# askerlee/AdaFace-dev

Measured on AMD Instinct MI355X. Metric: denoise-steps/sec SD-1.5 U-Net 512px bs=4/GPU, higher is better.
Workload: dtype f16; 1 GPU; adaface_txt2img_ddim: SD-1.5 U-Net eps-prediction + CFG + DDIM update, 512x512 (latent 64x64), bs=4/GPU, U-Net batch 8 (cond+uncond), 77 tokens, DDIM-50 timesteps, random-init weights; parallelism=replicas x1, hipgraph=True, finite=True

## Files before the change

adaface-dev_amd/_lib.py:

```python
import ctypes as C
import os
import subprocess

_HERE = os.path.dirname(os.path.abspath(__file__))
CSRC = os.path.join(_HERE, "csrc")
LIB_PATH = os.environ.get("AF_LIB") or os.path.join(CSRC, "libadaface_hip.so")

AF_OK, AF_E_BADARG, AF_E_UNSUPPORTED, AF_E_HIP = 0, -1, -2, -3
AF_ACT_NONE, AF_ACT_SILU, AF_ACT_GEGLU, AF_ACT_QUICKGELU = 0, 1, 2, 3
AF_OUT_NORMAL, AF_OUT_SPLIT_T, AF_OUT_F32 = 0, 1, 2
AF_SPLITK_COUNTER_BYTES = 4096 * 4
AF_FAM_GEMM, AF_FAM_ATTN, AF_FAM_GNORM, AF_FAM_LNORM, AF_FAM_ELEM, AF_FAM_XATTN = 0, 1, 2, 3, 4, 5

EXPORTS = (
    "af_last_error", "af_version", "af_device_count", "af_prof_enable", "af_prof_reset", "af_prof_read",
    "af_gemm", "af_groupnorm_ws_floats", "af_groupnorm", "af_layernorm", "af_attention", "af_attention_scores",
    "af_timestep_embedding", "af_nchw_f32_to_nhwc_f16", "af_nhwc_f16_to_nchw_f32", "af_cfg_ddim_step", "af_q_sample",
    "af_silu_f16", "af_attention_lse", "af_groupnorm_stats", "af_attention_bwd_scratch_bytes", "af_attention_bwd",
    "af_groupnorm_bwd", "af_layernorm_bwd", "af_geglu_fwd", "af_geglu_bwd", "af_sumpool2x2", "af_add_f16",
    "af_transpose_tokens", "af_cadamw_step", "af_attention_ex", "af_colsum", "af_quickgelu_fwd", "af_quickgelu_bwd",
    "af_scale_f32", "af_affine_prelu", "af_maxpool2x2", "af_global_avgpool", "af_se_residual_prelu", "af_axpy_f16", "af_dora_combine", "af_mul_f16", "af_im2col3x3", "af_colsum_tall", "af_softmax_rows", "af_attention_strided", "af_clamp_f32", "af_mask_pairs", "af_prefetch", "af_prefetch_ex",
    "af_xattn_scores", "af_xattn_softmax_pv", "af_xattn_softmax_pv_bwd", "af_xattn_rowmix", "af_xattn_colmix_ws_bytes", "af_xattn_colmix",
    "af_layernorm_param_grads", "af_transpose_tokens_pair", "af_ff_fused", "af_ff_chain", "af_xattn_fused",
    "af_softmax_rows_bwd", "af_affine_prelu_bwd", "af_maxpool2x2_bwd", "af_se_gate_grad", "af_se_residual_prelu_bwd",
    "af_groupnorm_apply", "af_gemm_gn_stats_ok", "af_gemm_halo_variant", "af_gn_proj_fused",
    "af_splitk_reduce", "af_groupnorm_splitk_ok", "af_groupnorm_splitk", "af_xattn_chain",
    "af_image_u8_to_nhwc_f16", "af_vae_latents_q_sample", "af_cfg_dpmpp_step", "af_cfg_lcm_step",
    "af_cfg_ddim_inpaint_step", "af_cfg_dpmpp_inpaint_step", "af_cfg_lcm_inpaint_step", "af_vae_latents_z_q_sample",
    "af_vae_attention", "af_latent_resize_q_sample", "af_affine_prelu_ch", "af_face_align_crop",
    "af_stem_im2col7x7", "af_relu_maxpool3x3s2", "af_subsample2x", "af_upsample2x_add", "af_retina_decode", "af_retina_nms",
)


class GemmDesc(C.Structure):
    _fields_ = [
        ("a1", C.c_void_p), ("a2", C.c_void_p), ("wt", C.c_void_p), ("bias", C.c_void_p),
        ("rowbias", C.c_void_p), ("residual", C.c_void_p), ("out", C.c_void_p), ("out2", C.c_void_p),
        ("M", C.c_int32), ("N", C.c_int32), ("K", C.c_int32), ("kpad", C.c_int32), ("taps", C.c_int32),
        ("c1", C.c_int32), ("c2", C.c_int32), ("lda1", C.c_int32), ("lda2", C.c_int32),
        ("B", C.c_int32), ("H", C.c_int32), ("W", C.c_int32), ("Ho", C.c_int32), ("Wo", C.c_int32),
        ("stride", C.c_int32), ("upsample", C.c_int32), ("rows_per_batch", C.c_int32), ("ld_rowbias", C.c_int32),
        ("act", C.c_int32), ("out_mode", C.c_int32), ("ld_out", C.c_int32), ("split_col", C.c_int32),
        ("ld_out2", C.c_int32), ("tile", C.c_int32), ("splits", C.c_int32),
        ("workspace", C.c_void_p), ("workspace_bytes", C.c_int64), ("zeros", C.c_void_p),
        ("tap_shift", C.c_int32), ("splitk_fused", C.c_int32),
        ("ln_colsum", C.c_void_p), ("ln_eps", C.c_float),
        ("a3", C.c_void_p), ("a4", C.c_void_p), ("c3", C.c_int32), ("c4", C.c_int32), ("lda3", C.c_int32), ("lda4", C.c_int32),
        ("gn_partials", C.c_void_p), ("gn_cpg", C.c_int32),
        ("defer_reduce", C.POINTER(C.c_int32)),
    ]


def _csrc_sha() -> str:
    import glob
    import hashlib
    h = hashlib.sha256()
    files = sorted(glob.glob(os.path.join(CSRC, "*.hip")) + glob.glob(os.path.join(CSRC, "*.h")))
    files += [os.path.join(CSRC, "Makefile"), os.path.join(os.path.dirname(_HERE), "include", "adaface_hip.h")]
    for f in files:
        h.update(os.path.basename(f).encode())
        with open(f, "rb") as fh:
            h.update(fh.read())
    return h.hexdigest()
# ... 25 lines not shown

_lib = None


def lib() -> C.CDLL:
    global _lib
    if _lib is not None:
        return _lib
    import torch
    if not os.path.exists(LIB_PATH):
        raise RuntimeError(
            f"{LIB_PATH} not found: the HIP extension is required (no CPU fallback). "
            "Run `python -c 'import __graft_entry__ as g; g.build()'` or `make -C adaface-dev_amd/csrc`."
        )
    L = C.CDLL(LIB_PATH)
    vp, i32, i64, f32 = C.c_void_p, C.c_int, C.c_int64, C.c_float
    L.af_last_error.restype = C.c_char_p
    L.af_last_error.argtypes = []
    L.af_version.argtypes = []
    L.af_device_count.argtypes = []
    L.af_prof_enable.argtypes = [i32]
    L.af_prof_reset.argtypes = []
    L.af_prof_read.argtypes = [i32, C.POINTER(C.c_int), C.POINTER(C.c_double)]
    L.af_gemm.argtypes = [C.POINTER(GemmDesc), vp]
    L.af_groupnorm_ws_floats.argtypes = [i32]
    L.af_groupnorm.argtypes = [vp, vp, i32, i32, vp, vp, vp, i32, i32, i32, f32, i32, vp, vp]
    L.af_groupnorm_apply.argtypes = [vp, i32, vp, vp, vp, vp, i32, i32, i32, f32, i32, vp, i32, vp]
    L.af_gemm_gn_stats_ok.argtypes = [i32, i32, i32, i32, i32, i32, i32, i32]
    L.af_gemm_halo_variant.argtypes = [C.POINTER(GemmDesc)]
    L.af_splitk_reduce.argtypes = [vp, i32, vp, vp, i32, i32, vp, vp, i32, i32, vp]
    L.af_groupnorm_splitk_ok.argtypes = [i32, i32, i32, i32]
    L.af_groupnorm_splitk.argtypes = [vp, i32, vp, vp, i32, vp, vp, i32, vp, vp, vp, vp, i32, i32, i32, f32, i32, vp]
    L.af_gn_proj_fused.argtypes = [vp, vp, i32, vp, vp, f32, vp, vp, i32, vp, i32, i32, i32, i32, vp, vp]
    L.af_layernorm.argtypes = [vp, vp, vp, vp, i32, i32, f32, vp]
    L.af_attention.argtypes = [vp, vp, vp, vp, vp, i32, i32, i32, i32, i32, i32, i32, i32, i32, i32, f32, vp]
    L.af_attention_scores.argtypes = [vp, vp, vp, vp, i32, i32, i32, i32, i32, f32, vp]
    L.af_timestep_embedding.argtypes = [vp, vp, i32, i32, f32, vp]
    L.af_nchw_f32_to_nhwc_f16.argtypes = [vp, vp, i32, i32, i32, i32, vp]
    L.af_nhwc_f16_to_nchw_f32.argtypes = [vp, vp, i32, i32, i32, i32, vp]
    L.af_cfg_ddim_step.argtypes = [vp, vp, vp, vp, i64, i32, f32, f32, f32, vp]
    L.af_cfg_dpmpp_step.argtypes = [vp, vp, vp, vp, vp, vp, i64, i32, f32, f32, f32, f32, f32, f32, vp]
    L.af_cfg_lcm_step.argtypes = [vp, vp, vp, vp, vp, i64, i32, f32, f32, f32, f32, f32, f32, f32, vp]
    L.af_q_sample.argtypes = [vp, vp, vp, vp, vp, i32, i64, vp]
    L.af_image_u8_to_nhwc_f16.argtypes = [vp, vp, i32, i32, i32, vp]
    L.af_vae_latents_q_sample.argtypes = [vp, vp, vp, vp, vp, f32, f32, f32, vp, i32, i32, i32, i32, vp]
    L.af_vae_latents_z_q_sample.argtypes = [vp, vp, vp, vp, vp, f32, f32, f32, vp, vp, i32, i32, i32, i32, vp]
    L.af_latent_resize_q_sample.argtypes = [vp, vp, vp, i32, i32, i32, i32, i32, i32, f32, f32, vp]
    blend = [vp, vp, vp, i32, i32, i64, f32, f32]
    L.af_cfg_ddim_inpaint_step.argtypes = L.af_cfg_ddim_step.argtypes[:-1] + blend + [vp]
    L.af_cfg_dpmpp_inpaint_step.argtypes = L.af_cfg_dpmpp_step.argtypes[:-1] + blend + [vp]
    L.af_cfg_lcm_inpaint_step.argtypes = L.af_cfg_lcm_step.argtypes[:-1] + blend + [vp]
    L.af_silu_f16.argtypes = [vp, vp, i64, vp]
    L.af_attention_lse.argtypes = [vp, vp, vp, vp, vp, i32, vp, i32, i32, i32, i32, i32, i32, i32, i32, i32, i32, f32, vp]
    L.af_attention_ex.argtypes = [vp, vp, vp, vp, vp, i32, vp, i32, i32, i32, i32, i32, i32, i32, i32, i32, i32, i32, f32, vp]
    L.af_attention_strided.argtypes = [vp, vp, vp, vp, vp, i32, vp, i32, i32, i32, i32, i32, i32, i32, i32, i32, i32, i32, i64, f32, vp]
    L.af_groupnorm_stats.argtypes = [vp, vp, i32, i32, vp, vp, vp, vp, i32, i32, i32, f32, i32, vp, vp]
    L.af_attention_bwd_scratch_bytes.argtypes = [i32, i32, i32, i32, i32]
    L.af_attention_bwd.argtypes = [vp, vp, vp, vp, vp, vp, i32, vp, i32, vp, vp, vp, vp, i64] + [i32] * 14 + [f32, vp]
    L.af_axpy_f16.argtypes = [vp, vp, f32, vp, i64, vp]
    L.af_dora_combine.argtypes = [vp, vp, vp, vp, vp, vp, i64, i32, vp]
    L.af_mul_f16.argtypes = [vp, vp, vp, i64, vp]
    L.af_im2col3x3.argtypes = [vp, vp, i32, i32, i32, i32, i32, vp]
    L.af_softmax_rows.argtypes = [vp, vp, i64, i32, vp]
    L.af_mask_pairs.argtypes = [vp, vp, i32, vp]
    L.af_vae_attention.argtypes = [vp, vp, vp, vp, i32, i32, i32, i32, i32, i32, i32, vp]
    L.af_prefetch.argtypes = [vp, i64, vp]
# ... 58 lines not shown
```

adaface-dev_amd/ldm/modules/diffusionmodules/openaimodel.py:

```python
import os
from abc import abstractmethod

import torch
import torch.nn as nn

from .... import ops
from ....ops import AF_ACT_SILU, F16
from ..attention import SpatialTransformer
from .util import (_PackCache, checkpoint, conv_nd, from_nhwc_f16, linear, normalization, timestep_embedding,
                   to_nhwc_f16, zero_module)


class TimestepBlock(nn.Module):
    @abstractmethod
    def forward(self, x, emb):
        """Apply the module to `x` given `emb` timestep embeddings."""


FUSE_SKIP = os.environ.get("AF_FUSE_SKIP", "1") != "0"


class SkipCat(tuple):
    """(h, skip): the decoder's channel concat, kept as two tensors so consumers read both
    sources directly instead of materialising torch.cat (openaimodel.py:918)."""


class EmbPack:

    def __init__(self, silu_emb, all_out=None):
        self.silu_emb = silu_emb
        self.all_out = all_out


class TimestepEmbedSequential(nn.Sequential, TimestepBlock):
    def hip(self, x, emb, context=None, mask=None):
        n = len(self)
        for i, layer in enumerate(self):
            if isinstance(layer, ResBlock):
                x = layer.hip(x, emb, defer_out=i + 1 < n and isinstance(self[i + 1], SpatialTransformer))
            elif isinstance(layer, TimestepBlock):
                x = layer.hip(x, emb)
            elif isinstance(layer, SpatialTransformer):
                x = layer.hip(x, context, mask)
            else:
                x = layer.hip(x)
        return x

    def hip_train(self, x, emb, context=None, mask=None):
        saved = []
        for layer in self:
            if isinstance(layer, TimestepBlock):
                x, s = layer.hip_train(x, emb)
# ... 349 lines not shown
        ca_idx = self.ALL_CA_LAYER_INDICES if ca_layer_indices is None else ca_layer_indices
        tr_idx = self.ALL_CA_LAYER_INDICES if trans_layer_indices is None else trans_layer_indices
        return apply(ca_flag_dict, ca_idx, "ca"), apply(trans_flag_dict, tr_idx, "trans")

    def _packed_emb_all(self):
        params = []
        for rb in self._resblocks:
            params += [rb.emb_layers[1].weight, rb.emb_layers[1].bias]

        def build():
            dev = params[0].device
            K = self._resblocks[0].emb_channels
            w = torch.zeros((self._emb_total, K), dtype=torch.float32, device=dev)
            b = torch.zeros((self._emb_total,), dtype=torch.float32, device=dev)
            for rb in self._resblocks:
                off, width = rb._emb_slice
                w[off:off + width] = rb.emb_layers[1].weight.detach().float()
                b[off:off + width] = rb.emb_layers[1].bias.detach().float()
            return ops.pack_matrix(w, b, dev)

        return self._emb_cache.get(params, build)

    def prepare(self):
        for m in self.modules():
            if hasattr(m, "packed"):
                m.packed()
            if hasattr(m, "_packed_qkv") and m.to_k.in_features == m.to_q.in_features:
                m._packed_qkv()
            if hasattr(m, "_packed_kv") and m.to_k.in_features != m.to_q.in_features:
                m._packed_kv()
        self._packed_emb_all()
        return self

    def hip(self, x_nhwc, timesteps, context, img_mask=None, capture_layers=()):
        emb = self._embed(timesteps)
        kv_layers = self._project_context_all(context)
        try:
            return self._hip_blocks(x_nhwc, emb, context, img_mask, capture_layers)
        finally:
            for m in kv_layers:
                m._kv_pre = None

    def _cross_attn_layers(self):
        out = []
        for blocks in (self.input_blocks, [self.middle_block], self.output_blocks):
            for module in blocks:
                for layer in module:
                    if isinstance(layer, SpatialTransformer):
                        out += [tb.attn2 for tb in layer.transformer_blocks]
        return out

    def _project_context_all(self, context):
        layers = self._cross_attn_layers()
        if not layers or context is None:
            return []
        ws = [m.to_k.weight for m in layers] + [m.to_v.weight for m in layers]
        if not hasattr(self, "_kv_all_cache"):
            self._kv_all_cache = _PackCache()
        pack = self._kv_all_cache.get(ws, lambda: ops.pack_matrix(torch.cat([w.detach() for w in ws], 0), None, ws[0].device))
        B, L, cc = context.shape
        sc = pack.N // 2
        k_all, vt_all = ops.gemm(context.reshape(B * L, cc), pack, rows_per_batch=L, split_col=sc)
        off = 0
        for m in layers:
            c = m.inner_dim
            m._kv_pre = (k_all[:, off:off + c], vt_all[:, off:off + c, :], sc)
            off += c
        return layers

    def _hip_blocks(self, x_nhwc, emb, context, img_mask, capture_layers):
        acts = {}
        hs = []
        h = x_nhwc
        layer_idx = 0

        def collect(module, h):
            attn2 = module[1].transformer_blocks[0].attn2
            a = attn2.cached_activations
            a["outfeat"] = from_nhwc_f16(h, torch.float32)
            acts[layer_idx] = a
            attn2.cached_activations = None

        for module in self.input_blocks:
            h = module.hip(h, emb, context, img_mask)
            hs.append(h)
            if layer_idx in capture_layers:
                collect(module, h)
            layer_idx += 1
        h = self.middle_block.hip(h, emb, context, img_mask)
        if layer_idx in capture_layers:
            collect(self.middle_block, h)
        layer_idx += 1
        for module in self.output_blocks:
            h = module.hip(SkipCat((h, hs.pop())), emb, context, img_mask)
            if layer_idx in capture_layers:
                collect(module, h)
            layer_idx += 1
        h = self.out[0].hip(h, silu=True)
        return self.out[2].hip(h), acts

    def hip_tail(self, trunk, timesteps, context, capture_layers, n_tail=3):
        h, skips = trunk
        emb = self._embed(timesteps)
        kv_layers = self._project_context_all(context)
        acts = {}
        try:
            n_out = len(self.output_blocks)
            layer_idx = len(self.input_blocks) + 1 + n_out - n_tail
            for k, module in enumerate(list(self.output_blocks)[n_out - n_tail:]):
                h = module.hip(SkipCat((h, skips[k])), emb, context, None)
                if layer_idx in capture_layers:
                    attn2 = module[1].transformer_blocks[0].attn2
                    a = attn2.cached_activations
                    a["outfeat"] = from_nhwc_f16(h, torch.float32)
                    acts[layer_idx] = a
                    attn2.cached_activations = None
                layer_idx += 1
            h = self.out[0].hip(h, silu=True)
            return self.out[2].hip(h), acts
        finally:
            for m in kv_layers:
                m._kv_pre = None

    def _embed(self, timesteps):
        t_emb = timestep_embedding(timesteps, self.model_channels)
        e0 = ops.gemm(t_emb, self.time_embed[0].packed(), act=AF_ACT_SILU)
        semb = ops.gemm(e0, self.time_embed[2].packed(), act=AF_ACT_SILU)
        return EmbPack(semb, ops.gemm(semb, self._packed_emb_all()))

    def hip_train(self, x_nhwc, timesteps, context, img_mask=None):
        emb = self._embed(timesteps)
        saved_in, saved_out, hs = [], [], []
        h = x_nhwc
        for module in self.input_blocks:
            h, s = module.hip_train(h, emb, context, img_mask)
            saved_in.append(s)
            hs.append(h)
        h, saved_mid = self.middle_block.hip_train(h, emb, context, img_mask)
        for module in self.output_blocks:
            h, s = module.hip_train(SkipCat((h, hs.pop())), emb, context, img_mask)
            saved_out.append(s)
        g, st = self.out[0].hip_train(h, silu=True)
        return self.out[2].hip(g), (saved_in, saved_mid, saved_out, h, st, context.shape)

    def hip_train_trunk(self, x_nhwc, emb, context, img_mask, n_tail):
        saved_in, saved_out, hs = [], [], []
        h = x_nhwc
        for module in self.input_blocks:
            h, s = module.hip_train(h, emb, context, img_mask)
            saved_in.append(s)
            hs.append(h)
        h, saved_mid = self.middle_block.hip_train(h, emb, context, img_mask)
# ... 58 lines not shown
            scaled = res_gradscale != 1.0 and (n_out - 1 - i) >= self.num_res_blocks + 1
            d = ops.axpy(d, dskips[i], res_gradscale) if scaled else ops.add(d, dskips[i])
            if i == 0 and not need_dx:
                return None, dctx.reshape(ctx_shape)
            d, dctx = self.input_blocks[i].hip_bwd(saved_in[i], d, dctx)
        return d, dctx.reshape(ctx_shape)

    def forward(self, x, timesteps=None, context=None, y=None, context_in=None, extra_info=None, **kwargs):
        assert y is None, "must specify y if and only if the model is class-conditional"
        capture = extra_info.get("capture_ca_activations", False) if extra_info is not None else False
        img_mask = extra_info.get("img_mask", None) if extra_info is not None else None
        captured = [22, 23, 24] if capture else []
        old_flags = None
        if capture:
            old_flags, _ = self.set_cross_attn_flags(ca_flag_dict={"save_cross_attn_vars": True}, ca_layer_indices=captured)
        ei = extra_info or {}
        rewrites = bool(ei.get("normalize_cross_attn", False) or ei.get("mix_attn_mats_in_batch", False))
        trainable = torch.is_grad_enabled() and (x.requires_grad or context.requires_grad or ei.get("_ffn_lora_adapters")
                                                 or ei.get("_attn_lora_adapters"))
        if rewrites or ei.get("_attn_lora_adapters") or (capture and trainable):
            from .capture_graph import unet_forward_captured
            if extra_info is None:
                raise ValueError("extra_info must be a dict on the capture / score-rewrite path")
            if capture:
                self.set_cross_attn_flags(ca_flag_dict=old_flags, ca_layer_indices=captured)
            eps = unet_forward_captured(self, x, timesteps, context, extra_info)
            if not capture:
                extra_info.pop("ca_layers_activations", None)
            return eps
        if trainable:
            gs = float((extra_info or {}).get("res_hidden_states_gradscale", 1) or 1)
            lora = (extra_info or {}).get("_ffn_lora_adapters")
            return _UNetFunction.apply(self, x, timesteps, context, img_mask, gs, lora, *[t[3] for t in lora_param_order(lora)])
        try:
            ctx = context.to(F16).contiguous()
            shared = None
            if img_mask is None and ei.get("_trunk_cache") is not None:
                from .capture_graph import cached_trunk
                shared = cached_trunk(ei, x.shape[0])
            if shared is not None:
                eps, acts = self.hip_tail(shared, timesteps, ctx, captured)
            else:
                xh = to_nhwc_f16(x, ops.round_up(self.in_channels, 8))
                eps, acts = self.hip(xh, timesteps, ctx, img_mask, captured)
        finally:
            if capture:
                self.set_cross_attn_flags(ca_flag_dict=old_flags, ca_layer_indices=captured)
        if extra_info is not None:
            extra_info["ca_layers_activations"] = {
                key: {li: acts[li][key] for li in acts} for key in ("outfeat", "attn", "attnscore", "q", "q2", "k", "v", "attn_out")
            }
        return from_nhwc_f16(eps, x.dtype, self.out_channels)


class _UNetFunction(torch.autograd.Function):

    @staticmethod
    def forward(ctx, unet, x, timesteps, context, img_mask, res_gradscale=1.0, lora=None, *lora_params):
        ctx.res_gradscale = res_gradscale
        ctx.lora = lora
        ctx.need_dx, ctx.x_dtype, ctx.c_dtype = x.requires_grad, x.dtype, context.dtype

        def body(xs, ts, cs, ms):
            xh = to_nhwc_f16(xs, ops.round_up(unet.in_channels, 8))
            try:
                for bi, ads in (lora or {}).items():
                    unet.output_blocks[bi][0]._lora = ads
                eps, saved = unet.hip_train(xh, ts, cs.to(F16).contiguous(), ms)
            finally:
                for bi in (lora or {}):
                    unet.output_blocks[bi][0]._lora = None
            return from_nhwc_f16(eps, xs.dtype, unet.out_channels), saved

        graphs = getattr(unet, "train_graphs", None)
        if graphs is not None and x.is_cuda:
            ctx.key = (tuple(x.shape), tuple(context.shape), str(x.dtype), str(context.dtype), img_mask is not None, float(res_gradscale),
                       tuple(id(a) for _, _, _, a in lora_param_order(lora)), ctx.need_dx)
            from_graph = not graphs[0].busy(ctx.key) and graphs[0].entries.get(ctx.key, {}).get("state") in ("warm", "graph")
            out, ctx.saved = graphs[0].run(ctx.key, body, [x.detach(), timesteps, context.detach(), img_mask],
                                           refresh=lambda: _refresh_adapter_packs(lora))
            if not from_graph:
                ctx.key = None
            elif any(ctx.needs_input_grad):
                graphs[0].claim(ctx.key, ctx)
# ... 54 lines not shown
```

adaface-dev_amd/ops.py:

```python
import ctypes as C
from dataclasses import dataclass
from typing import Optional

import torch

from . import _lib
from ._lib import AF_ACT_GEGLU, AF_ACT_NONE, AF_ACT_QUICKGELU, AF_ACT_SILU, AF_OUT_F32, AF_OUT_NORMAL, AF_OUT_SPLIT_T, GemmDesc

F16 = torch.float16
NEG_MAX = -torch.finfo(torch.float32).max



def param_key(p):
    if p is None:
        return None
    gen = p.__dict__.get("_af_gen")
    return (p.data_ptr(), p._version, p.device, gen[0] if gen is not None else -1)


def _stream() -> int:
    return torch._C._cuda_getCurrentRawStream(torch._C._cuda_getDevice())


# ... 576 lines not shown
        rc = _lib.lib().af_groupnorm(_p(x), _p(x2), c1, c2, _p(gamma), _p(beta), _p(y), B, hw, groups, float(eps), int(silu), _p(ws), _stream())
        _lib.check(rc, "af_groupnorm")
    else:
        rc = _lib.lib().af_groupnorm_stats(_p(x), _p(x2), c1, c2, _p(gamma), _p(beta), _p(y), _p(stats), B, hw, groups, float(eps), int(silu), _p(ws), _stream())
        _lib.check(rc, "af_groupnorm_stats")
    return y, stats


def groupnorm(x: torch.Tensor, gamma: torch.Tensor, beta: torch.Tensor, eps: float, silu: bool, *,
              x2: Optional[torch.Tensor] = None, groups: int = 32) -> torch.Tensor:
    return _groupnorm(x, gamma, beta, eps, silu, x2, groups, False)[0]


def groupnorm_train(x, gamma, beta, eps, silu, *, x2=None, groups=32):
    return _groupnorm(x, gamma, beta, eps, silu, x2, groups, True)


def gn_proj_fused(x: torch.Tensor, gamma: torch.Tensor, beta: torch.Tensor, eps: float, pw: PackedWeight, groups: int = 32) -> Optional[torch.Tensor]:
    gn = partials_of(x)
    B, c = x.shape[0], x.shape[-1]
    hw = x.numel() // (B * c)
    if (gn is None or c != 320 or groups != 32 or pw.N != 320 or pw.K != 320 or pw.ln_cs is not None or hw % 128 != 0 or gn.B != B or gn.hw != hw or gn.C != c
            or gn.cpg * groups != c or not x.is_contiguous()):
        return None
    _chk_f16(x, "gn_proj_fused.x")
    out = torch.empty((B * hw, pw.N), dtype=F16, device=x.device)
    _pf_note(pw.wt)
    rc = _lib.lib().af_gn_proj_fused(_p(x), _p(gn.ws), gn.nblk, _p(gamma), _p(beta), float(eps), _p(pw.wt), _p(pw.bias), pw.kpad, _p(out), B, hw, c, groups,
                                     _zero_page(x.device).data_ptr(), _stream())
    _lib.check(rc, "af_gn_proj_fused")
    return out


def layernorm(x: torch.Tensor, gamma: torch.Tensor, beta: torch.Tensor, eps: float = 1e-5) -> torch.Tensor:
    _chk_f16(x, "layernorm.x")
    Cn = x.shape[-1]
    y = torch.empty_like(x)
    _lib.check(_lib.lib().af_layernorm(_p(x), _p(gamma), _p(beta), _p(y), x.numel() // Cn, Cn, float(eps), _stream()),
               "af_layernorm")
    return y


def attention(q: torch.Tensor, k: torch.Tensor, vt: torch.Tensor, *, B: int, Nq: int, L: int, heads: int, d: int,
              ldq: int, ldk: int, keybias: Optional[torch.Tensor] = None, scale: Optional[float] = None,
              want_lse: bool = False, causal_m: int = 0):
    Cn = heads * d
    o = torch.empty((B * Nq, Cn), dtype=F16, device=q.device)
    scale = d ** -0.5 if scale is None else scale
    ldb = 0 if keybias is None else keybias.stride(0)
    lse = torch.empty((B, heads, round_up(Nq, 32)), dtype=torch.float32, device=q.device) if want_lse else None
    rc = _lib.lib().af_attention_strided(_p(q), _p(k), _p(vt), _p(o), _p(lse), 0 if lse is None else lse.stride(1), _p(keybias),
                                         int(causal_m), B, Nq, L, heads, d, ldq, ldk, Cn, vt.stride(1), ldb, vt.stride(0), float(scale),
                                         _stream())
    _lib.check(rc, "af_attention")
    return (o, lse) if want_lse else o


_attn_scratch = {}


def attention_bwd(q, k, v, o, dout, lse, *, B: int, Nq: int, L: int, heads: int, d: int, ldq: int, ldk: int, ldv: int,
                  dq: torch.Tensor, dk: torch.Tensor, dv: torch.Tensor, lddq: int, lddk: int, lddv: int,
                  keybias: Optional[torch.Tensor] = None, scale: Optional[float] = None, causal_m: int = 0):
    Cn = heads * d
    scale = d ** -0.5 if scale is None else scale
    need = _lib.lib().af_attention_bwd_scratch_bytes(B, Nq, L, heads, d)
# ... 631 lines not shown
```

include/adaface_hip.h:

```cpp
#ifndef ADAFACE_HIP_H
#define ADAFACE_HIP_H

#include <stdint.h>

#ifdef __cplusplus
extern "C" {
#endif

#define AF_OK 0
#define AF_E_BADARG (-1)
#define AF_E_UNSUPPORTED (-2)
#define AF_E_HIP (-3)

const char* af_last_error(void);
int af_version(void);
int af_device_count(void);

#define AF_FAM_GEMM 0
#define AF_FAM_ATTN 1
#define AF_FAM_GNORM 2
#define AF_FAM_LNORM 3
#define AF_FAM_ELEM 4
#define AF_FAM_XATTN 5
#define AF_FAM_COUNT 6
// ... 47 lines not shown
  const void* a4;
  int32_t c3, c4, lda3, lda4;
  void* gn_partials;
  int32_t gn_cpg;
  int32_t* defer_reduce;
} af_gemm_desc;
#define AF_SPLITK_MAX_TILES 4096
#define AF_SPLITK_COUNTER_BYTES (AF_SPLITK_MAX_TILES * 4)

int af_gemm(const af_gemm_desc* d, void* stream);

int af_splitk_reduce(const void* slabs, int splits, const void* bias, const void* rowbias, int ld_rowbias, int rows_per_batch, const void* residual,
                     void* out, int M, int N, void* stream);

int af_ff_fused(const void* x, const void* w1, const void* b1, const void* ln_colsum, float ln_eps, int kpad1, const void* w2, const void* b2,
                int kpad2, const void* residual, void* out, int M, int C, int inner, const void* zeros, void* stream);
int af_ff_chain(const void* x, const void* w1, const void* b1, const void* ln_colsum, float ln_eps, int kpad1, const void* w2, const void* b2, int kpad2,
                const void* residual, const void* wp, const void* bp, int kpad_p, const void* x_in, void* out, void* gn_partials, int gn_cpg,
                int rows_per_batch, int M, int C, int inner, const void* zeros, void* stream);

int af_xattn_fused(const void* x, const void* wq, const void* bq, const void* ln_colsum, float ln_eps, int kpad_q, const void* k, int ldk,
                   const void* vt, int64_t vt_batch_stride, int ldv, const void* wo, const void* bo, int kpad_o, const void* residual,
                   void* out, int B, int N, int L, int C, int heads, float scale, const void* zeros, void* stream);

int af_xattn_chain(const void* ao, const void* w1, const void* b1, int kpad_1, const void* x0, void* x1, const void* wq, const void* bq,
                   const void* ln_colsum, float ln_eps, int kpad_q, const void* k, int ldk, const void* vt, int64_t vt_batch_stride, int ldv,
                   const void* wo, const void* bo, int kpad_o, void* out, int B, int N, int L, int C, int heads, float scale, const void* zeros,
                   void* stream);


int af_gn_proj_fused(const void* x, const void* partials, int nblk, const void* gamma, const void* beta, float eps, const void* w, const void* bias,
                     int kpad, void* out, int B, int HW, int C, int groups, const void* zeros, void* stream);

int af_groupnorm_ws_floats(int B);
int af_groupnorm_apply(const void* x, int C, const void* gamma, const void* beta, void* y, void* stats, int B, int HW, int groups, float eps,
                       int silu, const void* partials, int nblk, void* stream);
int af_groupnorm_splitk_ok(int B, int HW, int C, int groups);
int af_groupnorm_splitk(const void* slabs, int splits, const void* bias, const void* rowbias, int ld_rowbias, const void* residual, void* x_out, int C,
                        const void* gamma, const void* beta, void* y, void* stats, int B, int HW, int groups, float eps, int silu, void* stream);
int af_gemm_gn_stats_ok(int tile, int splits, int taps, int act, int out_mode, int N, int cpg, int rows_per_batch);
int af_gemm_halo_variant(const af_gemm_desc* d);
int af_groupnorm(const void* x1, const void* x2, int c1, int c2, const void* gamma, const void* beta,
                 void* y, int B, int HW, int groups, float eps, int silu, void* workspace, void* stream);

int af_groupnorm_stats(const void* x1, const void* x2, int c1, int c2, const void* gamma, const void* beta,
                       void* y, void* stats, int B, int HW, int groups, float eps, int silu, void* workspace,
                       void* stream);

int af_layernorm(const void* x, const void* gamma, const void* beta, void* y, int rows, int C, float eps,
                 void* stream);

int af_attention(const void* q, const void* k, const void* vt, void* o, const void* keybias, int B, int Nq,
                 int L, int heads, int d, int ldq, int ldk, int ldo, int ldv, int ldb, float scale, void* stream);
int af_attention_lse(const void* q, const void* k, const void* vt, void* o, void* lse2, int ld_lse, const void* keybias,
                     int B, int Nq, int L, int heads, int d, int ldq, int ldk, int ldo, int ldv, int ldb, float scale,
                     void* stream);

int af_attention_ex(const void* q, const void* k, const void* vt, void* o, void* lse2, int ld_lse, const void* keybias,
                    int causal_m, int B, int Nq, int L, int heads, int d, int ldq, int ldk, int ldo, int ldv, int ldb,
                    float scale, void* stream);
int af_attention_strided(const void* q, const void* k, const void* vt, void* o, void* lse2, int ld_lse, const void* keybias, int causal_m,
                         int B, int Nq, int L, int heads, int d, int ldq, int ldk, int ldo, int ldv, int ldb, int64_t vt_batch_stride,
                         float scale, void* stream);

int64_t af_attention_bwd_scratch_bytes(int B, int Nq, int L, int heads, int d);
int af_attention_bwd(const void* q, const void* k, const void* v, const void* o, const void* dout, const void* lse2,
// ... 115 lines not shown
```

Before: 96.63 denoise-steps/s.

## Fuse U-Net input conv with layout conversion and output GroupNorm+SiLU+conv head

Adds two new HIP kernels. The first fuses the final GroupNorm+SiLU+3x3 conv (C to 4) and optionally writes NCHW f32 directly, dropping the separate norm pass, conv launch and layout conversion. The second fuses the NCHW f32 to NHWC f16 conversion with the first 3x3 conv (4 to 320) and emits GroupNorm partials for the next layer. Together they remove several small launches and intermediate tensors at both ends of each U-Net step, but rely on bespoke MFMA kernels with small per-block work that may underuse the GPU.

```diff
diff --git a/adaface-dev_amd/_lib.py b/adaface-dev_amd/_lib.py
--- a/adaface-dev_amd/_lib.py
+++ b/adaface-dev_amd/_lib.py
@@ -29,6 +29,7 @@
     "af_cfg_ddim_inpaint_step", "af_cfg_dpmpp_inpaint_step", "af_cfg_lcm_inpaint_step", "af_vae_latents_z_q_sample",
     "af_vae_attention", "af_latent_resize_q_sample", "af_affine_prelu_ch", "af_face_align_crop",
     "af_stem_im2col7x7", "af_relu_maxpool3x3s2", "af_subsample2x", "af_upsample2x_add", "af_retina_decode", "af_retina_nms",
+    "af_out_head_fused", "af_in_head_fused",
 )
 
 
@@ -120,6 +121,8 @@
     L.af_groupnorm_splitk_ok.argtypes = [i32, i32, i32, i32]
     L.af_groupnorm_splitk.argtypes = [vp, i32, vp, vp, i32, vp, vp, i32, vp, vp, vp, vp, i32, i32, i32, f32, i32, vp]
     L.af_gn_proj_fused.argtypes = [vp, vp, i32, vp, vp, f32, vp, vp, i32, vp, i32, i32, i32, i32, vp, vp]
+    L.af_out_head_fused.argtypes = [vp, vp, i32, vp, vp, f32, vp, vp, i32, vp, i32, i32, i32, i32, i32, i32, vp]
+    L.af_in_head_fused.argtypes = [vp, i32, vp, vp, i32, vp, vp, i32, i32, i32, i32, i32, vp]
     L.af_layernorm.argtypes = [vp, vp, vp, vp, i32, i32, f32, vp]
     L.af_attention.argtypes = [vp, vp, vp, vp, vp, i32, i32, i32, i32, i32, i32, i32, i32, i32, i32, f32, vp]
     L.af_attention_scores.argtypes = [vp, vp, vp, vp, i32, i32, i32, i32, i32, f32, vp]
diff --git a/adaface-dev_amd/csrc/af_step_fused.hip b/adaface-dev_amd/csrc/af_step_fused.hip
--- /dev/null
+++ b/adaface-dev_amd/csrc/af_step_fused.hip
@@ -0,0 +1,338 @@
+#include "af_common.h"
+
+namespace {
+
+constexpr int SF_NBLK = 128, SF_MAXG = 32;
+
+__device__ __forceinline__ half8_t sf_zero8() { return half8_t{0, 0, 0, 0, 0, 0, 0, 0}; }
+
+constexpr int OH_T = 8, OH_HP = OH_T + 2, OH_NPIX = OH_HP * OH_HP, OH_PD = 8, OH_U = 8;
+constexpr int OH_MAX_C = 640;
+constexpr int OH_TAIL_FLOATS = 8 * SF_MAXG * 3 + SF_MAXG * 2 + 4 * 64 * 4;
+
+__host__ __device__ constexpr int oh_lds_bytes(int C) { return OH_NPIX * (C * 2 + 16) + 2 * C * 4 + OH_TAIL_FLOATS * 4; }
+
+struct OhArgs {
+  const half_t* x;
+  const float* ws;
+  const float* gamma;
+  const float* beta;
+  const half_t* w;
+  const float* bias;
+  void* out;
+  int nblk, kpad, out_nchw_f32;
+  int B, H, W, C, groups, cpg, tiles_x;
+  float eps;
+};
+
+__global__ __launch_bounds__(256) void af_out_head_kernel(const OhArgs a) {
+  extern __shared__ __attribute__((aligned(16))) char af_smem[];
+  const int C = a.C, CP = C >> 3, stride = C * 2 + 16;
+  char* act = af_smem;
+  float* sc = reinterpret_cast<float*>(af_smem + OH_NPIX * stride);
+  float* sh = sc + C;
+  float* fold = sh + C;
+  float* mr = fold + 8 * SF_MAXG * 3;
+  float* red = mr + SF_MAXG * 2;
+  const int t = threadIdx.x, lane = t & 63, wave = t >> 6;
+  const int b = blockIdx.y, ty = blockIdx.x / a.tiles_x, tx = blockIdx.x - ty * a.tiles_x;
+  const int y0 = ty * OH_T - 1, x0 = tx * OH_T - 1, HW = a.H * a.W;
+  const int total = OH_NPIX * CP;
+  const half_t* xb = a.x + (size_t)b * HW * C;
+
+  half8_t v[OH_U];
+  auto src = [&](int idx) -> int {
+    if (idx >= total) return -1;
+    const int pix = idx / CP, ch = idx - pix * CP;
+    const int hy = pix / OH_HP, hx = pix - hy * OH_HP;
+    const int gy = y0 + hy, gx = x0 + hx;
+    if (gy < 0 || gy >= a.H || gx < 0 || gx >= a.W) return -1;
+    return (gy * a.W + gx) * C + ch * 8;
+  };
+  auto issue = [&](int base) {
+#pragma unroll
+    for (int u = 0; u < OH_U; ++u) {
+      const int o = src(base + u * 256 + t);
+      if (o >= 0) v[u] = *reinterpret_cast<const half8_t*>(xb + o);
+    }
+  };
+  issue(0);
+  {
+    const int g = t & 31, kl = t >> 5;
+    GnAcc acc = {0.f, 0.f, 0.f};
+    if (g < a.groups) {
+      const float* wsb = a.ws + (size_t)b * SF_NBLK * SF_MAXG * 2;
+      const int per = (HW + a.nblk - 1) / a.nblk;
+      for (int k = kl; k < a.nblk; k += 8) {
+        const float* w = wsb + ((size_t)k * SF_MAXG + g) * 2;
+        const int cnt = min(HW, (k + 1) * per) - k * per;
+        GnAcc pk;
+        pk.n = cnt > 0 ? (float)cnt * (float)a.cpg : 0.f;
+        pk.s = w[0];
+        pk.m2 = w[1];
+        acc = gn_acc_merge(acc, pk);
+      }
+    }
+    fold[(kl * SF_MAXG + g) * 3 + 0] = acc.n;
+    fold[(kl * SF_MAXG + g) * 3 + 1] = acc.s;
+    fold[(kl * SF_MAXG + g) * 3 + 2] = acc.m2;
+  }
+  __syncthreads();
+  if (t < a.groups) {
+    GnAcc acc = {fold[t * 3], fold[t * 3 + 1], fold[t * 3 + 2]};
+#pragma unroll
+    for (int k = 1; k < 8; ++k) acc = gn_acc_merge(acc, GnAcc{fold[(k * SF_MAXG + t) * 3], fold[(k * SF_MAXG + t) * 3 + 1], fold[(k * SF_MAXG + t) * 3 + 2]});
+    const float inv_n = 1.0f / ((float)HW * (float)a.cpg);
+    mr[t * 2] = acc.s * inv_n;
+    mr[t * 2 + 1] = rsqrtf(fmaxf(acc.m2 * inv_n, 0.f) + a.eps);
+  }
+  __syncthreads();
+  for (int c = t; c < C; c += 256) {
+    const int g = c / a.cpg;
+    const float k = mr[g * 2 + 1] * a.gamma[c];
+    sc[c] = k;
+    sh[c] = a.beta[c] - mr[g * 2] * k;
+  }
+  __syncthreads();
+  for (int base = 0; base < total; base += 256 * OH_U) {
+    if (base) issue(base);
+#pragma unroll
+    for (int u = 0; u < OH_U; ++u) {
+      const int idx = base + u * 256 + t;
+      if (idx < total) {
+        const int pix = idx / CP, ch = idx - pix * CP;
+        half8_t o = sf_zero8();
+        if (src(idx) >= 0) {
+          const floatx4 s0 = *reinterpret_cast<const floatx4*>(sc + ch * 8), s1 = *reinterpret_cast<const floatx4*>(sc + ch * 8 + 4);
+          const floatx4 h0 = *reinterpret_cast<const floatx4*>(sh + ch * 8), h1 = *reinterpret_cast<const floatx4*>(sh + ch * 8 + 4);
+#pragma unroll
+          for (int e = 0; e < 8; ++e) {
+            const float f = (float)v[u][e] * (e < 4 ? s0[e & 3] : s1[e & 3]) + (e < 4 ? h0[e & 3] : h1[e & 3]);
+            o[e] = (half_t)af_silu(f);
+          }
+        }
+        *reinterpret_cast<half8_t*>(act + pix * stride + ch * 16) = o;
+      }
+    }
+  }
+  __syncthreads();
+
+  const int nch = C >> 5, nunits = 9 * nch;
+  const int nn = lane & 15, nq = lane >> 4;
+  const int n_w = (nunits - wave + 3) >> 2;
+  auto wload = [&](int i) -> half8_t {
+    const int u = wave + 4 * i;
+    const int tap = u / nch, c32 = u - tap * nch;
+    if (nn >= 4) return sf_zero8();
+    return *reinterpret_cast<const half8_t*>(a.w + (size_t)nn * a.kpad + tap * C + c32 * 32 + nq * 8);
+  };
+  half8_t ring[OH_PD];
+#pragma unroll
+  for (int j = 0; j < OH_PD; ++j) ring[j] = j < n_w ? wload(j) : sf_zero8();
+  floatx4 acc[4];
+#pragma unroll
+  for (int g = 0; g < 4; ++g) acc[g] = floatx4{0.f, 0.f, 0.f, 0.f};
+  for (int i0 = 0; i0 < n_w; i0 += OH_PD) {
+#pragma unroll
+    for (int j = 0; j < OH_PD; ++j) {
+      const int i = i0 + j;
+      if (i < n_w) {
+        const half8_t wf = ring[j];
+        if (i + OH_PD < n_w) ring[j] = wload(i + OH_PD);
+        const int u = wave + 4 * i;
+        const int tap = u / nch, c32 = u - tap * nch;
+        const int ky = tap / 3, kx = tap - ky * 3;
+#pragma unroll
+        for (int g = 0; g < 4; ++g) {
+          const int p = g * 16 + nn;
+          const half8_t xf = *reinterpret_cast<const half8_t*>(act + (((p >> 3) + ky) * OH_HP + (p & 7) + kx) * stride + (c32 * 32 + nq * 8) * 2);
+          acc[g] = __builtin_amdgcn_mfma_f32_16x16x32_f16(wf, xf, acc[g], 0, 0, 0);
+        }
+      }
+    }
+  }
+  if (nq == 0) {
+#pragma unroll
+    for (int g = 0; g < 4; ++g) *reinterpret_cast<floatx4*>(red + (wave * 64 + g * 16 + nn) * 4) = acc[g];
+  }
+  __syncthreads();
+  {
+    const int n = t >> 6, p = t & 63;
+    float s = a.bias ? a.bias[n] : 0.f;
+#pragma unroll
+    for (int w = 0; w < 4; ++w) s += red[(w * 64 + p) * 4 + n];
+    const int gy = ty * OH_T + (p >> 3), gx = tx * OH_T + (p & 7);
+    if (gy < a.H && gx < a.W) {
+      const half_t hv = (half_t)s;
+      if (a.out_nchw_f32) reinterpret_cast<float*>(a.out)[(((size_t)b * 4 + n) * a.H + gy) * a.W + gx] = (float)hv;
+      else reinterpret_cast<half_t*>(a.out)[(((size_t)b * a.H + gy) * a.W + gx) * 4 + n] = hv;
+    }
+  }
+}
+
+constexpr int IH_KL = 104;
+constexpr int IH_MAX_N = 320;
+
+__host__ __device__ constexpr int ih_lds_bytes(int N) { return N * IH_KL * 2 + 128 * (N + 8) * 2 + 2 * N * 4; }
+
+struct IhArgs {
+  const float* x;
+  const half_t* w;
+  const float* bias;
+  half_t* out;
+  float* ws;
+  int B, Cin, H, W, HW, N, kpad, cpg, groups;
+};
+
+__global__ __launch_bounds__(512) void af_in_head_kernel(const IhArgs a) {
+  extern __shared__ __attribute__((aligned(16))) char af_smem[];
+  const int N = a.N, lo = N + 8;
+  half_t* wl = reinterpret_cast<half_t*>(af_smem);
+  half_t* ot = wl + N * IH_KL;
+  float* cs = reinterpret_cast<float*>(ot + 128 * lo);
+  float* cq = cs + N;
+  const int t = threadIdx.x, lane = t & 63, wave = t >> 6, nn = lane & 15, nq = lane >> 4;
+  const int b = blockIdx.y, blk = blockIdx.x, p0 = blk * 128;
+
+  half8_t xf[3];
+  {
+    const int p = p0 + wave * 16 + nn, y = p / a.W, x = p - y * a.W;
+#pragma unroll
+    for (int s = 0; s < 3; ++s) {
+      xf[s] = sf_zero8();
+      const int tap = 4 * s + nq;
+      const int ky = tap / 3, kx = tap - ky * 3;
+      const int gy = y + ky - 1, gx = x + kx - 1;
+      if (tap < 9 && gy >= 0 && gy < a.H && gx >= 0 && gx < a.W) {
+#pragma unroll
+        for (int c = 0; c < 8; ++c)
+          if (c < a.Cin) xf[s][c] = (half_t)a.x[((size_t)(b * a.Cin + c) * a.H + gy) * a.W + gx];
+      }
+    }
+  }
+  for (int idx = t; idx < N * 12; idx += 512) {
+    const int row = idx / 12, ch = idx - row * 12;
+    *reinterpret_cast<half8_t*>(wl + row * IH_KL + ch * 8) = *reinterpret_cast<const half8_t*>(a.w + (size_t)row * a.kpad + ch * 8);
+  }
+  __syncthreads();
+  for (int cg = 0; cg < N; cg += 64) {
+    half8_t o[2];
+#pragma unroll
+    for (int j = 0; j < 4; ++j) {
+      const int nrow = cg + 16 * (nn >> 2) + 4 * j + (nn & 3);
+      floatx4 acc = {0.f, 0.f, 0.f, 0.f};
+#pragma unroll
+      for (int s = 0; s < 3; ++s)
+        acc = __builtin_amdgcn_mfma_f32_16x16x32_f16(*reinterpret_cast<const half8_t*>(wl + nrow * IH_KL + (4 * s + nq) * 8), xf[s], acc, 0, 0, 0);
+#pragma unroll
+      for (int r = 0; r < 4; ++r) o[j >> 1][(j & 1) * 4 + r] = (half_t)(acc[r] + (a.bias ? a.bias[cg + 16 * nq + 4 * j + r] : 0.f));
+    }
+    half_t* dst = ot + (wave * 16 + nn) * lo + cg + 16 * nq;
+    *reinterpret_cast<half8_t*>(dst) = o[0];
+    *reinterpret_cast<half8_t*>(dst + 8) = o[1];
+  }
+  __syncthreads();
+  if (a.ws) {
+    for (int c = t; c < N; c += 512) {
+      const float pv = (float)ot[c];
+      float ss = 0.f, qq = 0.f;
+#pragma unroll 16
+      for (int px = 0; px < 128; ++px) {
+        const float f = (float)ot[px * lo + c] - pv;
+        ss += f;
+        qq += f * f;
+      }
+      cs[c] = ss;
+      cq[c] = qq;
+    }
+    __syncthreads();
+    if (t < a.groups) {
+      const float n = 128.f, P = (float)ot[t * a.cpg];
+      float ss = 0.f, qq = 0.f;
+      for (int c = t * a.cpg; c < (t + 1) * a.cpg; ++c) {
+        const float d = (float)ot[c] - P;
+        ss += cs[c] + n * d;
+        qq += cq[c] + 2.f * d * cs[c] + n * d * d;
+      }
+      const GnAcc acc = gn_acc_from_shifted(n * (float)a.cpg, P, ss, qq);
+      float* w = a.ws + (((size_t)b * SF_NBLK + blk) * SF_MAXG + t) * 2;
+      w[0] = acc.s;
+      w[1] = acc.m2;
+    }
+  }
+  const int NP = N >> 3;
+  half_t* ob = a.out + ((size_t)b * a.HW + p0) * N;
+  for (int idx = t; idx < 128 * NP; idx += 512) {
+    const int px = idx / NP, ch = idx - px * NP;
+    *reinterpret_cast<half8_t*>(ob + (size_t)px * N + ch * 8) = *reinterpret_cast<const half8_t*>(ot + px * lo + ch * 8);
+  }
+}
+
+}
+
+extern "C" int af_out_head_fused(const void* x, const void* partials, int nblk, const void* gamma, const void* beta, float eps, const void* w, const void* bias,
+                                 int kpad, void* out, int out_nchw_f32, int B, int H, int W, int C, int groups, void* stream) {
+  AF_REQUIRE(x && partials && gamma && beta && w && out, "af_out_head_fused: null pointer");
+  AF_REQUIRE(B > 0 && H > 0 && W > 0 && B <= 65535 && (long)H * W * C < (1L << 31), "af_out_head_fused: bad sizes");
+  AF_SUPPORTED(C % 32 == 0 && C <= OH_MAX_C, "af_out_head_fused: C must be a multiple of 32, at most 640");
+  AF_REQUIRE(groups > 0 && groups <= SF_MAXG && C % groups == 0, "af_out_head_fused: groups must divide C and be <= 32");
+  AF_REQUIRE(nblk > 0 && nblk <= SF_NBLK, "af_out_head_fused: nblk must be 1 .. 128");
+  AF_REQUIRE(kpad >= 9 * C && kpad % 8 == 0, "af_out_head_fused: the weight row stride must cover 9 C and be a multiple of 8");
+  AF_REQUIRE((((uintptr_t)x | (uintptr_t)w | (uintptr_t)gamma | (uintptr_t)beta) & 15) == 0, "af_out_head_fused: x / w / gamma / beta must be 16-byte aligned");
+  OhArgs a;
+  a.x = (const half_t*)x;
+  a.ws = (const float*)partials;
+  a.gamma = (const float*)gamma;
+  a.beta = (const float*)beta;
+  a.w = (const half_t*)w;
+  a.bias = (const float*)bias;
+  a.out = out;
+  a.nblk = nblk;
+  a.kpad = kpad;
+  a.out_nchw_f32 = out_nchw_f32;
+  a.B = B;
+  a.H = H;
+  a.W = W;
+  a.C = C;
+  a.groups = groups;
+  a.cpg = C / groups;
+  a.tiles_x = (W + OH_T - 1) / OH_T;
+  a.eps = eps;
+  const int tiles_y = (H + OH_T - 1) / OH_T;
+  static bool attr_set = false;
+  if (!af_allow_dyn_lds(reinterpret_cast<const void*>(&af_out_head_kernel), oh_lds_bytes(OH_MAX_C), attr_set, "af_out_head_fused")) return af_check_launch("af_out_head_fused");
+  AfLaunchScope scope(AF_FAM_GEMM, stream);
+  hipLaunchKernelGGL(af_out_head_kernel, dim3(a.tiles_x * tiles_y, B), dim3(256), oh_lds_bytes(C), (hipStream_t)stream, a);
+  return af_check_launch("af_out_head_fused");
+}
+
+extern "C" int af_in_head_fused(const void* x_nchw_f32, int Cin, const void* w, const void* bias, int kpad, void* out, void* partials, int groups, int B, int H,
+                                int W, int N, void* stream) {
+  AF_REQUIRE(x_nchw_f32 && w && out, "af_in_head_fused: null pointer");
+  AF_REQUIRE(B > 0 && B <= 65535 && H > 0 && W > 0 && Cin > 0 && (long)B * Cin * H * W < (1L << 31), "af_in_head_fused: bad sizes");
+  AF_SUPPORTED(Cin <= 8 && N > 0 && N % 64 == 0 && N <= IH_MAX_N, "af_in_head_fused: Cin <= 8, N a multiple of 64, at most 320");
+  AF_SUPPORTED((H * W) % 128 == 0 && H * W / 128 <= SF_NBLK, "af_in_head_fused: H W must be a multiple of 128, at most 128 blocks");
+  AF_REQUIRE(kpad >= 96 && kpad % 8 == 0, "af_in_head_fused: the weight row stride must be a multiple of 8, at least 96");
+  AF_REQUIRE(!partials || (groups > 0 && groups <= SF_MAXG && N % groups == 0), "af_in_head_fused: groups must divide N and be <= 32");
+  AF_REQUIRE((((uintptr_t)w | (uintptr_t)out) & 15) == 0, "af_in_head_fused: w / out must be 16-byte aligned");
+  IhArgs a;
+  a.x = (const float*)x_nchw_f32;
+  a.w = (const half_t*)w;
+  a.bias = (const float*)bias;
+  a.out = (half_t*)out;
+  a.ws = (float*)partials;
+  a.B = B;
+  a.Cin = Cin;
+  a.H = H;
+  a.W = W;
+  a.HW = H * W;
+  a.N = N;
+  a.kpad = kpad;
+  a.groups = partials ? groups : 0;
+  a.cpg = partials ? N / groups : 0;
+  static bool attr_set = false;
+  if (!af_allow_dyn_lds(reinterpret_cast<const void*>(&af_in_head_kernel), ih_lds_bytes(IH_MAX_N), attr_set, "af_in_head_fused")) return af_check_launch("af_in_head_fused");
+  AfLaunchScope scope(AF_FAM_GEMM, stream);
+  hipLaunchKernelGGL(af_in_head_kernel, dim3(a.HW / 128, B), dim3(512), ih_lds_bytes(N), (hipStream_t)stream, a);
+  return af_check_launch("af_in_head_fused");
+}
diff --git a/adaface-dev_amd/ldm/modules/diffusionmodules/openaimodel.py b/adaface-dev_amd/ldm/modules/diffusionmodules/openaimodel.py
--- a/adaface-dev_amd/ldm/modules/diffusionmodules/openaimodel.py
+++ b/adaface-dev_amd/ldm/modules/diffusionmodules/openaimodel.py
@@ -18,6 +18,8 @@
 
 
 FUSE_SKIP = os.environ.get("AF_FUSE_SKIP", "1") != "0"
+FUSE_OUT_HEAD = os.environ.get("AF_FUSE_OUT_HEAD", "1") != "0"
+FUSE_IN_HEAD = os.environ.get("AF_FUSE_IN_HEAD", "1") != "0"
 
 
 class SkipCat(tuple):
@@ -433,11 +435,11 @@
         self._packed_emb_all()
         return self
 
-    def hip(self, x_nhwc, timesteps, context, img_mask=None, capture_layers=()):
+    def hip(self, x_nhwc, timesteps, context, img_mask=None, capture_layers=(), eps_nchw_f32=False, h0=None):
         emb = self._embed(timesteps)
         kv_layers = self._project_context_all(context)
         try:
-            return self._hip_blocks(x_nhwc, emb, context, img_mask, capture_layers)
+            return self._hip_blocks(x_nhwc, emb, context, img_mask, capture_layers, eps_nchw_f32, h0)
         finally:
             for m in kv_layers:
                 m._kv_pre = None
@@ -469,7 +471,23 @@
             off += c
         return layers
 
-    def _hip_blocks(self, x_nhwc, emb, context, img_mask, capture_layers):
+    def _head(self, h, nchw_f32=False):
+        norm, conv = self.out[0], self.out[2]
+        if FUSE_OUT_HEAD and conv.kernel_size == (3, 3) and conv.stride == (1, 1) and norm.weight.dtype == torch.float32:
+            eps = ops.out_head_fused(h, norm.weight, norm.bias, norm.eps, conv.packed(), norm.num_groups, nchw_f32=nchw_f32)
+            if eps is not None:
+                return eps
+        eps = conv.hip(norm.hip(h, silu=True))
+        return ops.nhwc_f16_to_nchw_f32(eps, self.out_channels) if nchw_f32 else eps
+
+    def _in_head(self, x):
+        blk = self.input_blocks[0]
+        conv = blk[0] if len(blk) == 1 else None
+        if not FUSE_IN_HEAD or not isinstance(conv, nn.Conv2d) or conv.kernel_size != (3, 3) or conv.stride != (1, 1) or getattr(conv, "cin_pad", 0) != 8:
+            return None
+        return ops.in_head_fused(x, conv.packed())
+
+    def _hip_blocks(self, x_nhwc, emb, context, img_mask, capture_layers, eps_nchw_f32=False, h0=None):
         acts = {}
         hs = []
         h = x_nhwc
@@ -483,7 +501,7 @@
             attn2.cached_activations = None
 
         for module in self.input_blocks:
-            h = module.hip(h, emb, context, img_mask)
+            h = h0 if (layer_idx == 0 and h0 is not None) else module.hip(h, emb, context, img_mask)
             hs.append(h)
             if layer_idx in capture_layers:
                 collect(module, h)
@@ -497,10 +515,9 @@
             if layer_idx in capture_layers:
                 collect(module, h)
             layer_idx += 1
-        h = self.out[0].hip(h, silu=True)
-        return self.out[2].hip(h), acts
-
-    def hip_tail(self, trunk, timesteps, context, capture_layers, n_tail=3):
+        return self._head(h, eps_nchw_f32), acts
+
+    def hip_tail(self, trunk, timesteps, context, capture_layers, n_tail=3, eps_nchw_f32=False):
         h, skips = trunk
         emb = self._embed(timesteps)
         kv_layers = self._project_context_all(context)
@@ -517,8 +534,7 @@
                     acts[layer_idx] = a
                     attn2.cached_activations = None
                 layer_idx += 1
-            h = self.out[0].hip(h, silu=True)
-            return self.out[2].hip(h), acts
+            return self._head(h, eps_nchw_f32), acts
         finally:
             for m in kv_layers:
                 m._kv_pre = None
@@ -643,6 +659,7 @@
             gs = float((extra_info or {}).get("res_hidden_states_gradscale", 1) or 1)
             lora = (extra_info or {}).get("_ffn_lora_adapters")
             return _UNetFunction.apply(self, x, timesteps, context, img_mask, gs, lora, *[t[3] for t in lora_param_order(lora)])
+        f32_out = x.dtype != F16
         try:
             ctx = context.to(F16).contiguous()
             shared = None
@@ -650,10 +667,11 @@
                 from .capture_graph import cached_trunk
                 shared = cached_trunk(ei, x.shape[0])
             if shared is not None:
-                eps, acts = self.hip_tail(shared, timesteps, ctx, captured)
+                eps, acts = self.hip_tail(shared, timesteps, ctx, captured, eps_nchw_f32=f32_out)
             else:
-                xh = to_nhwc_f16(x, ops.round_up(self.in_channels, 8))
-                eps, acts = self.hip(xh, timesteps, ctx, img_mask, captured)
+                h0 = self._in_head(x)
+                xh = to_nhwc_f16(x, ops.round_up(self.in_channels, 8)) if h0 is None else None
+                eps, acts = self.hip(xh, timesteps, ctx, img_mask, captured, eps_nchw_f32=f32_out, h0=h0)
         finally:
             if capture:
                 self.set_cross_attn_flags(ca_flag_dict=old_flags, ca_layer_indices=captured)
@@ -661,6 +679,8 @@
             extra_info["ca_layers_activations"] = {
                 key: {li: acts[li][key] for li in acts} for key in ("outfeat", "attn", "attnscore", "q", "q2", "k", "v", "attn_out")
             }
+        if f32_out:
+            return eps if x.dtype == torch.float32 else eps.to(x.dtype)
         return from_nhwc_f16(eps, x.dtype, self.out_channels)
 
 
diff --git a/adaface-dev_amd/ops.py b/adaface-dev_amd/ops.py
--- a/adaface-dev_amd/ops.py
+++ b/adaface-dev_amd/ops.py
@@ -632,6 +632,42 @@
     return out
 
 
+def out_head_fused(x: torch.Tensor, gamma: torch.Tensor, beta: torch.Tensor, eps: float, pw: PackedWeight, groups: int = 32, *,
+                   nchw_f32: bool = False) -> Optional[torch.Tensor]:
+    gn = partials_of(x)
+    if gn is None or x.dim() != 4 or not x.is_contiguous():
+        return None
+    B, H, W, c = x.shape
+    if (pw.N != 4 or pw.taps != 9 or pw.cin != c or pw.k_tail or pw.ln_cs is not None or c % 32 or c > 640 or groups > 32 or c % groups or B > 65535
+            or H * W * c >= 1 << 31 or gn.B != B or gn.hw != H * W or gn.C != c or gn.cpg * groups != c or gamma.data_ptr() % 16 or beta.data_ptr() % 16):
+        return None
+    _chk_f16(x, "out_head_fused.x")
+    out = torch.empty((B, 4, H, W), dtype=torch.float32, device=x.device) if nchw_f32 else torch.empty((B, H, W, 4), dtype=F16, device=x.device)
+    _pf_note(pw.wt)
+    rc = _lib.lib().af_out_head_fused(_p(x), _p(gn.ws), gn.nblk, _p(gamma), _p(beta), float(eps), _p(pw.wt), _p(pw.bias), pw.kpad, _p(out), int(nchw_f32),
+                                      B, H, W, c, groups, _stream())
+    _lib.check(rc, "af_out_head_fused")
+    return out
+
+
+def in_head_fused(x: torch.Tensor, pw: PackedWeight, groups: int = 32) -> Optional[torch.Tensor]:
+    if x.dim() != 4 or x.dtype != torch.float32 or not x.is_cuda or not x.is_contiguous():
+        return None
+    B, cin, H, W = x.shape
+    N = pw.N
+    if (pw.taps != 9 or pw.cin != 8 or cin > 8 or pw.k_tail or pw.ln_cs is not None or pw.kpad < 96 or N % 64 or N > 320 or (H * W) % 128 or H * W // 128 > 128
+            or B > 65535 or N % groups or groups > 32):
+        return None
+    out = torch.empty((B, H, W, N), dtype=F16, device=x.device)
+    gn = GnPartials.alloc(x.device, B, H * W, N, N // groups) if GN_FROM_PRODUCER else None
+    _pf_note(pw.wt)
+    rc = _lib.lib().af_in_head_fused(_p(x), cin, _p(pw.wt), _p(pw.bias), pw.kpad, _p(out), None if gn is None else _p(gn.ws), groups, B, H, W, N, _stream())
+    _lib.check(rc, "af_in_head_fused")
+    if gn is not None:
+        gn.attach(out)
+    return out
+
+
 def layernorm(x: torch.Tensor, gamma: torch.Tensor, beta: torch.Tensor, eps: float = 1e-5) -> torch.Tensor:
     _chk_f16(x, "layernorm.x")
     Cn = x.shape[-1]
diff --git a/include/adaface_hip.h b/include/adaface_hip.h
--- a/include/adaface_hip.h
+++ b/include/adaface_hip.h
@@ -103,6 +103,12 @@
 int af_gn_proj_fused(const void* x, const void* partials, int nblk, const void* gamma, const void* beta, float eps, const void* w, const void* bias,
                      int kpad, void* out, int B, int HW, int C, int groups, const void* zeros, void* stream);
 
+int af_out_head_fused(const void* x, const void* partials, int nblk, const void* gamma, const void* beta, float eps, const void* w, const void* bias,
+                      int kpad, void* out, int out_nchw_f32, int B, int H, int W, int C, int groups, void* stream);
+
+int af_in_head_fused(const void* x_nchw_f32, int Cin, const void* w, const void* bias, int kpad, void* out, void* partials, int groups, int B, int H,
+                     int W, int N, void* stream);
+
 int af_groupnorm_ws_floats(int B);
 int af_groupnorm_apply(const void* x, int C, const void* gamma, const void* beta, void* y, void* stats, int B, int HW, int groups, float eps,
                        int silu, const void* partials, int nblk, void* stream);
```

Measured after the change: 96.86 denoise-steps/s (median of 6 runs). No clear change (+0.2%).
